# mahilab/mahi-mpc

Measured on AMD Instinct MI355X. Metric: MPC solves/sec (whole node), nx=4 N=30 batch, at 1/2/4/8 MI355X, higher is better.
Workload: dtype f64; 1 GPU; cfg#2: 2-link arm nx=4 nu=2, N=30, h=2 ms, cold-start SQP (exact or Gauss-Newton Hessian: config.hessian) to ||grad||<=1e-8, ||g||<=1e-10; batch_per_gpu=4096, global_batch=4096, horizon=30, kkt_solver=riccati (16 lanes per instance), hessian=exact (Lagrangian, IPOPT's default), init_states=reference cold start V = 0 (MMPC_INIT_ZERO: V not read)

## Files before the change

mahi-mpc_amd/csrc/mmpc.hip:

```cpp
#include <hip/hip_runtime.h>

#include <algorithm>
#include <atomic>
#include <cmath>
#include <cstdio>
#include <cstring>
#include <fstream>
#include <mutex>
#include <thread>
#include <sstream>
#include <string>
#include <type_traits>
#include <vector>

#include <dlfcn.h>
#include <rccl/rccl.h>

#include "../../include/mmpc.h"
#include "json_lite.h"
#include "adjoint_sweep.h"
#include "tangent_sweep.h"
#include "gain_sweep.h"
#include "group_launch.h"
#include "lane_launch.h"
// ... 591 lines not shown
        }
    }
    if (staged) {
        __syncthreads();
        const int64_t nb = B - b0 < I ? B - b0 : I;
        double* const dst = traj + b0 * N * 8;
        for (int t = threadIdx.x; t < nb * N * 8; t += kSynthThreads) dst[t] = so[t];
    }
}

inline unsigned grid1d(int64_t B, int threads) { return static_cast<unsigned>((B + threads - 1) / threads); }
inline unsigned synth_blocks(int64_t B, int N) {
    const int64_t I = N < kSynthThreads ? kSynthThreads / N : 1;
    return static_cast<unsigned>((B + I - 1) / I);
}

template <class F>
int with_model(int model_id, F&& f) {
#if MMPC_BUILTIN_MODELS
    if (model_id == MMPC_MODEL_TWO_LINK_ARM) return f(static_cast<TwoLinkArm*>(nullptr));
    if (model_id == MMPC_MODEL_EXO_ARM) return f(static_cast<ExoArm*>(nullptr));
#else
    if (model_id == MMPC_MODEL_USER) return f(static_cast<UserModel*>(nullptr));
#endif
    return fail(MMPC_ERR_UNSUPPORTED, "model not compiled into this library");
}
int model_nq(int model_id) {
    int nq = 0;
    with_model(model_id, [&](auto* m) {
        nq = std::remove_pointer_t<decltype(m)>::NQ;
        return MMPC_OK;
    });
    return nq;
}

mmpc_model_info with_horizon(const mmpc_model_info& mi, int N) {
    mmpc_model_info r = mi;
    r.num_shooting_nodes = N;
    r.num_v = mi.num_x * (N + 1) + mi.num_u * N;
    r.num_g = mi.num_x * N;
    return r;
}

int group_ws_doubles(const mmpc_model_info& mi, const KernelVariant& v) {
    return mmpc::group_ws_doubles(mi.num_x, mi.num_u, mi.num_shooting_nodes, v.ub, v.xb, false, v.mehr);
}
int lane_ws_doubles(const mmpc_model_info& mi, int nq, const KernelVariant& v) {
    return mmpc::lane_ws_doubles(mi.num_x, mi.num_u, nq, mi.num_shooting_nodes, v.xb);
}
size_t group_lds_instance_bytes(const mmpc_model_info& mi, int nq, const KernelVariant& v) {
    const int kc = mi.model_id == MMPC_MODEL_TWO_LINK_ARM ? mmpc::GroupLaneOps<TwoLinkArm>::doubles
                   : mi.model_id == MMPC_MODEL_EXO_ARM    ? mmpc::GroupLaneOps<ExoArm>::doubles
                                                          : 0;
    return static_cast<size_t>(mmpc::group_lds_doubles(mi.num_x, mi.num_u, nq, mi.num_shooting_nodes, v.ub,
                                                       mi.is_linear != 0, v.xb, kc)) * sizeof(double);
}
size_t group_lds_bytes(const mmpc_model_info& mi, int nq, const KernelVariant& v) {
    return group_lds_instance_bytes(mi, nq, v) * kGroupsPerWave;
}
constexpr size_t kMaxGroupLds = 160 * 1024;

size_t solver_workspace_bytes(const mmpc_model_info& mi, int nq, int64_t B) {
    const size_t lane = static_cast<size_t>(lane_ws_doubles(mi, nq, kVariantXb)) * 64u *
                        static_cast<size_t>((B + 63) / 64) * sizeof(double);
    const size_t group = static_cast<size_t>(std::max(group_ws_doubles(mi, kVariantUb),
                                                      group_ws_doubles(mi, kVariantXbMehrotra))) *
                         static_cast<size_t>(B) * sizeof(double);
    return (std::max(lane, group) + 255) / 256 * 256;
}

int resolve_kkt_solver_base(const mmpc_handle* h, int64_t B) {
    const mmpc_model_info& mi = h->info;
    if (h->opts.kkt_solver != MMPC_KKT_AUTO) return h->opts.kkt_solver;
    if (h->opts.factor_fp32) return MMPC_KKT_RICCATI;
    const int N = mi.num_shooting_nodes;
    const size_t glds = group_lds_bytes(mi, h->nq, h->x_bounded ? kVariantXb : kVariantUb);
    if (mi.model_id == MMPC_MODEL_USER) {
        if (glds <= kMaxGroupLds / 2 && B * static_cast<int64_t>(N) <= 1000000) return MMPC_KKT_RICCATI_GROUP;
        return MMPC_KKT_RICCATI;
    }
    if (mi.model_id == MMPC_MODEL_TWO_LINK_ARM) {
        if (N * TwoLinkArm::NU <= 64 && B <= 2560 && (h->opts.hessian == MMPC_HESSIAN_GAUSS_NEWTON || mi.is_linear))
            return MMPC_KKT_CONDENSED;
        if (glds <= kMaxGroupLds && B * static_cast<int64_t>(N) <= 1000000) return MMPC_KKT_RICCATI_GROUP;
        return MMPC_KKT_RICCATI;
    }
    if (glds <= kMaxGroupLds / 2 && B <= 4096) return MMPC_KKT_RICCATI_GROUP;
    return MMPC_KKT_RICCATI;
}
int resolve_kkt_solver(const mmpc_handle* h, int64_t B) {
    const int s = resolve_kkt_solver_base(h, B);
    if (h->x_bounded && h->opts.kkt_solver == MMPC_KKT_AUTO && s == MMPC_KKT_CONDENSED)
        return group_lds_bytes(h->info, h->nq, kVariantXb) <= kMaxGroupLds ? MMPC_KKT_RICCATI_GROUP : MMPC_KKT_RICCATI;
    return s;
}

template <class M>
constexpr bool exact_capable() {
    return HasHess<M>::value && (M::NX + M::NU < kGroupLanes);
}
template <class M, class = void>
struct ExactDefault {
    static constexpr bool value = true;
};
template <class M>
struct ExactDefault<M, std::enable_if_t<!M::kExactDefault || M::kExactDefault>> {
    static constexpr bool value = M::kExactDefault;
};
// ... 1826 lines not shown
```

mahi-mpc_amd/csrc/sqp_group.h:

```cpp
#undef MMPC_GROUP_PASS
#if defined(MMPC_GROUP_BODY_ONLY)
#define MMPC_GROUP_PASS 2
#elif !defined(MMPC_SQP_GROUP_H)
#define MMPC_SQP_GROUP_H
#define MMPC_GROUP_PASS 1
#else
#define MMPC_GROUP_PASS 0
#endif
#if MMPC_GROUP_PASS == 1
#include <type_traits>

#include "models.h"
#include "sqp_lane.h"
#include "sqp_wave.h"

namespace mmpc {

template <class Model>
__host__ __device__ constexpr bool w_struct_zero(int, int) { return false; }
template <>
__host__ __device__ constexpr bool w_struct_zero<TwoLinkArm>(int r, int j) { return (r == 0 && j >= 2) || (r >= 2 && (j == 0 || j >= 4)); }
template <class Model>
struct WPack {
    static constexpr int PK = 0, OVER = 0;
    __host__ __device__ static constexpr int col(int) { return 0; }
    __host__ __device__ static constexpr int idx(int, int) { return -1; }
};
template <>
struct WPack<TwoLinkArm> {
    static constexpr int PK = 10, OVER = 3;
    __host__ __device__ static constexpr int col(int i) { return i < 3 ? i : 2 * (i - 1); }
    __host__ __device__ static constexpr int idx(int r, int j) {
        if (w_struct_zero<TwoLinkArm>(r, j)) return -1;
        return col(r) + col(j);
    }
};
template <class Model>
__host__ __device__ constexpr bool wpack_valid() {
    using P = WPack<Model>;
    constexpr int NX = Model::NX, KZ = Model::NX + Model::NU;
    for (int r = 0; r < NX; ++r)
        for (int j = 0; j < KZ; ++j) {
            if (P::idx(r, j) < 0) continue;
            if (P::idx(r, j) >= P::PK || P::idx(r, j) != P::col(r) + P::col(j)) return false;
            for (int r2 = 0; r2 < NX; ++r2)
                for (int j2 = 0; j2 < KZ; ++j2)
                    if (P::idx(r2, j2) == P::idx(r, j) && !((r2 == r && j2 == j) || (r2 == j && j2 == r))) return false;
        }
    return P::OVER == P::col(NX - 1) + P::col(KZ - 1) - (P::PK - 1);
}
static_assert(wpack_valid<TwoLinkArm>(), "W record of the 2-link arm");
template <class Model>
__host__ __device__ constexpr int wpack_col_rep(int j) {
    for (int q = 0; q < j; ++q) {
        bool same = true;
        for (int r = 0; r < Model::NX; ++r) same = same && ((WPack<Model>::idx(r, q) < 0) == (WPack<Model>::idx(r, j) < 0));
        if (same) return q;
    }
    return j;
}
constexpr int kGroupLanes = 16;
constexpr int kGroupsPerWave = 4;

__host__ __device__ constexpr int group_const_doubles(int nx, int nu) {
    return nx + nu < kGroupLanes ? nx + (nx > nu ? nx : nu) : 0;
}
__host__ __device__ constexpr int group_lds_doubles(int nx, int nu, int nq, int N, bool bounded = true,
                                                   bool linear = true, bool xb = false, int kc = 0) {
    return N * (3 * nx + (nx - nq) * (nq + (nx - nq) + nu) + 2 * nu) + 3 * (N + 1) * nx + (bounded ? N * nu : 0) +
           (linear ? (nx - nq) * (nq + (nx - nq) + nu) + nx : 0) +
           (N * ((nx - nq) * nu + nx) >= 2 * (nx - nq) * (nx - nq) ? 0 : 2 * (nx - nq) * (nx - nq)) + kc;
}
template <class Model>
struct GroupLaneOps {
    static constexpr int doubles = 0;
};
template <>
struct GroupLaneOps<TwoLinkArm> {
    static constexpr int doubles = group_const_doubles(TwoLinkArm::NX, TwoLinkArm::NU);
};
__host__ __device__ constexpr int group_hess_doubles(int nx, int nu) { return nx * (nx + nu) + nu * nu; }
__host__ __device__ constexpr int group_ws_doubles(int nx, int nu, int N, bool bounded = true, bool xb = false,
                                                  bool w_onchip = false, bool mehr = false) {
    return N * nu * (nx + nu + 1) + (w_onchip ? 0 : N * group_hess_doubles(nx, nu)) +
           (bounded ? N * nu * (nx + 2 * nu + 1) : 0) + (xb ? 5 * N * (nx + nu) : 0) +
           (mehr ? 2 * N * (nx + nu) + N * ((2 + nu) * kGroupLanes + nu * (nu + 1) / 2 + nu) : 0);
}
static_assert(kGroupsPerWave * group_lds_doubles(4, 2, 2, 30, false, false, false, GroupLaneOps<TwoLinkArm>::doubles) * 8 <= 40960,
              "cfg#2 LDS budget");

struct GroupWork {
    double* ws;
};

template <int O>
__device__ __forceinline__ double row_ror(double v) {
    static_assert(O >= 1 && O < 16, "row rotation");
    return __builtin_amdgcn_update_dpp(v, v, 0x120 + O, 0xf, 0xf, true);
}
__device__ __forceinline__ double group_sum(double v) {
    v += row_ror<8>(v);
    v += row_ror<4>(v);
    v += row_ror<2>(v);
    v += row_ror<1>(v);
    return v;
}
__device__ __forceinline__ double group_min(double v) {
    v = fmin(v, row_ror<8>(v));
    v = fmin(v, row_ror<4>(v));
    v = fmin(v, row_ror<2>(v));
    v = fmin(v, row_ror<1>(v));
    return v;
}
__device__ __forceinline__ double group_max(double v) {
    v = fmax(v, row_ror<8>(v));
    v = fmax(v, row_ror<4>(v));
    v = fmax(v, row_ror<2>(v));
    v = fmax(v, row_ror<1>(v));
    return v;
}
__device__ __forceinline__ double group_bcast(double v, int base) { return __shfl(v, base); }
__device__ __forceinline__ int group_bcast_i(int v, int base) { return __shfl(v, base); }

template <int L>
__device__ __forceinline__ double row_bcast(double v) {
    static_assert(L >= 0 && L < 16, "row lane");
    return __builtin_amdgcn_update_dpp(v, v, 0x150 + L, 0xf, 0xf, true);
}
template <int B, int E, class F>
__device__ __forceinline__ void sfor(F&& f) {
    if constexpr (B < E) {
        f(std::integral_constant<int, B>{});
        sfor<B + 1, E>(static_cast<F&&>(f));
    }
}

template <class Model>
__device__ __forceinline__ void group_model(bool lin, const double* lFq, const double* lFqd, const double* lFu,
                                            const double* lxd, const double* lxs, const double* lus, const double* x,
                                            const double* u, double* xd, double* Fq, double* Fqd, double* Fu,
                                            bool jac) {
// ... 60 lines not shown
#pragma unroll
            for (int e = 0; e < W; ++e) {
#pragma unroll
                for (int i = 0; i < NQ; ++i) xd[e][i] = x[e][NQ + i];
#pragma unroll
                for (int i = 0; i < NA; ++i) xd[e][NQ + i] = xdw[NQ + i].v[e];
#pragma unroll
                for (int i = 0; i < NA * NQ; ++i) Fq[e][i] = fq[i].v[e];
#pragma unroll
                for (int i = 0; i < FD; ++i) Fqd[e][i] = fqd[i].v[e];
#pragma unroll
                for (int i = 0; i < FU; ++i) Fu[e][i] = fu[i].v[e];
            }
        } else {
            Model::eval(xw, uw, xdw);
#pragma unroll
            for (int e = 0; e < W; ++e)
#pragma unroll
                for (int i = 0; i < NX; ++i) xd[e][i] = xdw[i].v[e];
        }
    }
}

template <class Model, bool BOUNDED = false, bool XB = false, bool EXACT = false>
__global__ __launch_bounds__(64) void sqp_group_kernel(SolveParams p, GroupWork gw) {
    constexpr bool MEHR = false;
    constexpr bool IB = false;
#endif
#if MMPC_GROUP_PASS != 0
    static_assert(!(BOUNDED && XB), "the interior-point variant handles the control bounds itself");
    static_assert(!MEHR || XB, "the barrier rule belongs to the interior-point variant");
    constexpr int NX = Model::NX, NU = Model::NU, NQ = Model::NQ, NA = NX - NQ, NS = NX + NU, ND = NX + NU;
    constexpr int SQ = NA * NQ > 0 ? NA * NQ : 1;
    constexpr int FQ = NA * NQ, FD = NA * NA, FU = NA * NU;
    static_assert(NQ >= 0 && NA >= NQ, "x = [q; z] with qdot = z[0:NQ]");
    constexpr int G = kGroupLanes;
    extern __shared__ double shm[];
    const int gl = threadIdx.x & (G - 1);
    const int gi = threadIdx.x / G;
    [[maybe_unused]] const int lane0 = threadIdx.x;
    MMPC_PHASE_DECL
    const int gbase = gi * G;
    const int64_t slot = (int64_t)blockIdx.x * p.gpw + gi;
    const bool resume = p.tail_idx != nullptr;
    const bool valid = gi < p.gpw && slot < (resume ? (int64_t)min(*p.tail_count, p.tail_slots) : p.B);
    if (!valid) return;
    const int64_t inst = resume ? (int64_t)p.tail_idx[slot] : slot;
    const int64_t ii = inst;
    const int N = p.N;
    const int NV = NX * (N + 1) + NU * N;
    const double h = p.h;

    constexpr int KC = NX + NU < kGroupLanes ? GroupLaneOps<Model>::doubles : 0;
    double* const sX = shm + gi * group_lds_doubles(NX, NU, NQ, N, BOUNDED, p.is_linear != 0, XB, KC);
    double* const sU = sX + (N + 1) * NX;
    double* const sD = sU + N * NU;
    double* const sDX = sD + (N + 1) * NX;
    double* const sDU = sDX + (N + 1) * NX;
    double* const sF = sDU + N * NU;
    double* const sC = sF + N * NX;
    double* const sFq = sC + N * NX;
    double* const sFqd = sFq + N * FQ;
    double* const sFu = sFqd + N * FD;
    double* const sR = sFu + N * FU;
    double* const sHold = sR + N * NX;
    double* const sLin = sHold + (BOUNDED ? N * NU : 0);
    constexpr int NY = NX + NU;
    constexpr int PK = WPack<Model>::PK;
    constexpr bool WLDS = EXACT && !BOUNDED && !XB && IsControlAffine<Model>::value && PK >= NX && PK <= 2 * NX + NU;
    double* const wK = gw.ws + slot * (int64_t)group_ws_doubles(NX, NU, N, BOUNDED, XB, WLDS, MEHR);
    constexpr int KZ = NX + NU, HW = group_hess_doubles(NX, NU);
    double* const wH = wK + N * NU * (NS + 1);
    double* const sW = sD + NX;
    static_assert(!WLDS || WPack<Model>::OVER <= NX, "the over-read of the last W record stays inside sDU");
    if constexpr (WLDS) {
        if (gl < WPack<Model>::OVER) sW[N * PK + gl] = 0.0;
    }
    constexpr int NR = NS + NU + 1;
    double* const wRel = wH + N * HW;
    bool w_zeros_stored = false;
    double* const sZl = wRel;
    double* const sZu = sZl + N * NY;
    double* const sSg = sZu + N * NY;
    double* const sBb = sSg + N * NY;
    double* const sZg = sBb + N * NY;
    [[maybe_unused]] double* const sCl = sZg + N * NY;
    [[maybe_unused]] double* const sCu = sCl + N * NY;
    constexpr int VL = 2 + NU, VC = NU * (NU + 1) / 2, VS = VC + NU, VR = VL * G + VS;
    [[maybe_unused]] double* const sVr = sCu + N * NY;
    const double* const trg = p.traj + ii * (int64_t)N * NX;

    constexpr bool PAIR = HasWideEval<Model>::value && !BOUNDED && !XB;
    constexpr int WD = PAIR ? 2 : 1;
    constexpr int WA = WD, WJ = WD, WW = WD;
    const double* w = p.weights + ii * p.w_stride;
    double Q[NX], R[NU], Rm[NU], up[NU];
#pragma unroll
    for (int r = 0; r < NX; ++r) Q[r] = w[r];
#pragma unroll
    for (int c = 0; c < NU; ++c) {
        R[c] = w[NX + c];
        Rm[c] = w[NX + NU + c];
        up[c] = p.u_prev[ii * NU + c];
    }
    double lbv[NU], ubv[NU];
    load_bounds<NU, BOUNDED, IB>(p, inst, lbv, ubv);
    [[maybe_unused]] double px0[NX], pxv[WD][NX], puv[WD][NU], prv[WD][NX];
// ... 28 lines not shown
    if constexpr (PAIR) {
#pragma unroll
        for (int r = 0; r < NX; ++r) px0[r] = p.x0[ii * NX + r];
        pro_load(gl, pxv, puv, prv);
    }
    constexpr bool DIST = (NS < G);
    static_assert(!MEHR || DIST, "Mehrotra's rule: lane-distributed path");
    constexpr bool CAFF = IsControlAffine<Model>::value;
    static_assert(!EXACT || (DIST && HasHess<Model>::value), "exact Hessian: lane-distributed path, model eval_hess");
    const int r = gl;
    const bool lx = r < NX, lu = r >= NX && r < NS, la = r >= NQ && r < NX;
    const int rx = lx ? r : 0;
    const int ru = lu ? r - NX : 0;
    const int ta = la ? r - NQ : 0;
    const double Qr = lx ? w[rx] : 0.0;
    [[maybe_unused]] const double lqd = r < NQ ? 1.0 : 0.0, lad = la ? 1.0 : 0.0;
    const double lxf = lx ? 1.0 : 0.0;
    int wrow = 0;
#pragma unroll
    for (int r2 = 0; r2 < NX; ++r2)
        if (lx && r == r2) wrow = WPack<Model>::col(r2);
    double wm[KZ];
#pragma unroll
    for (int j = 0; j < KZ; ++j) {
        bool nz = false;
#pragma unroll
        for (int r2 = 0; r2 < NX; ++r2)
            if (lx && r == r2 && WPack<Model>::idx(r2, j) >= 0) nz = true;
        wm[j] = wpack_col_rep<Model>(j) < j ? wm[wpack_col_rep<Model>(j)] : (nz ? 1.0 : 0.0);
    }
    const int rq = r < NQ ? r : 0;
    const double Rr = lu ? w[NX + ru] : 0.0;
    double dgx[NS];
#pragma unroll
    for (int j = 0; j < NS; ++j) dgx[j] = (lx && j == r) ? 1.0 : 0.0;
    double lbr = -INFINITY, ubr = INFINITY;
#pragma unroll
    for (int c = 0; c < NU; ++c)
        if (lu && ru == c) {
            lbr = lbv[c];
            ubr = ubv[c];
        }
    double hq[NQ > 0 ? NQ : 1], hrow[NX], qoh[NX], rdg[NU];
#pragma unroll
    for (int z = 0; z < NQ; ++z) hq[z] = (r == NQ + z) ? h : 0.0;
#pragma unroll
    for (int j = 0; j < NX; ++j) {
        hrow[j] = (r < NQ && j == NQ + r) ? h : 0.0;
        qoh[j] = (j == r) ? Qr : 0.0;
    }
#pragma unroll
    for (int c = 0; c < NU; ++c) rdg[c] = (r == NX + c) ? R[c] : 0.0;
    constexpr bool LOPS = KC > 0;
    double* const sKc = sX + group_lds_doubles(NX, NU, NQ, N, BOUNDED, p.is_linear != 0, XB, KC) - KC;
    using LdsB = const __attribute__((address_space(3))) char*;
    using LdsD = const __attribute__((address_space(3))) double*;
    const LdsB shb = (LdsB)shm;
    auto lds = [](LdsB b) { return *(LdsD)b; };
    auto pin = [](LdsB& b) { asm volatile("" : "+v"(b)); };
    [[maybe_unused]] const LdsB iKc = shb + 8 * (int)(sKc - shm), iKz = iKc + 8 * NX;
    constexpr bool MIRROR = LOPS && NQ > 0 && NQ == NA && (NA - 1) * NA < KC;
    [[maybe_unused]] const double Qa = MIRROR ? w[rx] : Qr;
    [[maybe_unused]] const LdsB iAq =
        la ? shb + 8 * ((int)(sFq - shm) + ta * NQ) : ((r < NQ || MIRROR) ? iKc + 8 * ((NX - 1) - (NQ + rq)) : iKz);
    [[maybe_unused]] const int zAq = la ? 8 * FQ : 0, zAd = la ? 8 * FD : 0, zBr = la ? 8 * FU : 0;
    [[maybe_unused]] const LdsB iAd = la ? shb + 8 * ((int)(sFqd - shm) + ta * NA) : ((r < NQ || MIRROR) ? iAq + 8 * NQ : iKz);
    [[maybe_unused]] const LdsB iBr = la ? shb + 8 * ((int)(sFu - shm) + ta * NU) : iKz;
    constexpr bool ACOLP = LOPS && NQ == NA && (NA - 1) * NA < KC;
    static_assert(!MIRROR || ACOLP, "a mirrored lane reads row 0's column through the per-lane column address");
    [[maybe_unused]] const int zAc = (la || r < NQ) ? 8 * FD : 0;
    [[maybe_unused]] const LdsB iAc = la ? shb + 8 * ((int)(sFqd - shm) + ta) : (r < NQ ? shb + 8 * ((int)(sFq - shm) + rq) : iKc),
                                iAcN = iAc + (N - 1) * zAc;
    if constexpr (LOPS) {
        for (int i = gl; i < KC; i += G) sKc[i] = (i == NX - 1) ? h : 0.0;
    }
    if constexpr (PAIR) {
        const bool hold = p.init_hold != 0;
        for (int k0 = gl; k0 <= N; k0 += WD * G) {
            if (k0 != gl) pro_load(k0, pxv, puv, prv);
#pragma unroll
            for (int e = 0; e < WD; ++e) {
                const int k = pro_k(k0, e), ku = k < N ? k : N - 1;
#pragma unroll
                for (int r = 0; r < NX; ++r) sX[k * NX + r] = (k == 0 || hold) ? px0[r] : pxv[e][r];
#pragma unroll
                for (int c = 0; c < NU; ++c) sU[ku * NU + c] = puv[e][c];
#pragma unroll
                for (int r = 0; r < NX; ++r) sR[ku * NX + r] = prv[e][r];
            }
        }
    } else {
        const double* Vin = p.V + ii * (int64_t)NV;
        for (int k = gl; k <= N; k += G) {
#pragma unroll
            for (int r = 0; r < NX; ++r)
                sX[k * NX + r] = (k == 0 || p.init_hold) ? p.x0[ii * NX + r] : (p.init_zero ? 0.0 : Vin[k * ND + r]);
            if (k < N) {
#pragma unroll
                for (int c = 0; c < NU; ++c) {
                    const double v = p.init_zero ? 0.0 : Vin[k * ND + NX + c];
                    sU[k * NU + c] = BOUNDED ? proj(v, lbv[c], ubv[c]) : v;
                }
#pragma unroll
                for (int r = 0; r < NX; ++r) sR[k * NX + r] = trg[k * NX + r];
            }
        }
    }
// ... 709 lines not shown
                for (int c = 0; c < NU; ++c) {
                    double g = 0.0;
#pragma unroll
                    for (int s2 = 0; s2 < NA; ++s2) g = fma(sFu[k * FU + s2 * NU + c], sD[(k + 1) * NX + NQ + s2], g);
                    const double uk = sU[k * NU + c], um = k == 0 ? up[c] : sU[(k - 1) * NU + c];
                    g = fma(R[c], uk - um, fma(Rm[c], uk, g));
                    if (k < N - 1) g -= R[c] * (sU[(k + 1) * NU + c] - uk);
                    if constexpr (XB) g += sZg[k * NY + NX + c];
                    if constexpr (!BOUNDED) {
                        gmax = fmax(gmax, fabs(2.0 * g));
                    } else {
                        gmax = fmax(gmax, fabs(uk - proj(uk - 2.0 * g, lbv[c], ubv[c])));
                        sHold[k * NU + c] = (uk <= lbv[c] + beps && g > 0.0)   ? lbv[c]
                                            : (uk >= ubv[c] - beps && g < 0.0) ? ubv[c]
                                                                                : NAN;
                    }
                    nonfinite |= !isfinite(g);
                }
            }
        };
        auto backward_dist = [&](bool useW) {
            if constexpr (BOUNDED) {
                __builtin_amdgcn_fence(__ATOMIC_RELEASE, "workgroup");
                __builtin_amdgcn_fence(__ATOMIC_ACQUIRE, "workgroup");
            }
            double Prow[NS], pvr;
            [[maybe_unused]] LdsB jcol = iAcN;
            const double lxm = lx ? 1.0 : 0.0;
            struct Wb {
                double r[KZ], u[NU * NU];
            };
            Wb w0;
            auto load_w = [&](int k, Wb& b) {
#pragma unroll
                for (int j = 0; j < KZ; ++j)
                    b.r[j] = WLDS ? sW[k * PK + wrow + WPack<Model>::col(j)] : wH[k * HW + rx * KZ + j];
                if constexpr (!CAFF) {
#pragma unroll
                    for (int j = 0; j < NU * NU; ++j) b.u[j] = wH[k * HW + NX * KZ + j];
                }
            };
            if (EXACT && useW) {
                load_w(N - 1, w0);
            }
#pragma unroll
            for (int j = 0; j < NS; ++j) Prow[j] = j < NX ? qoh[j] : 0.0;
            pvr = Qr * (lx ? sX[N * NX + rx] - tr[(N - 1) * NX + rx] : 0.0);
            if constexpr (XB) {
                const double sgN = sSg[(N - 1) * NY + rx], bbN = sBb[(N - 1) * NY + rx];
#pragma unroll
                for (int j = 0; j < NX; ++j) Prow[j] = fma(dgx[j], sgN, Prow[j]);
                pvr = fma(lxm, bbN, pvr);
            }
            auto stage = [&](int k, auto last_c, Wb& wb) {
                constexpr bool LAST = decltype(last_c)::value;
#if defined(MMPC_PHASE_TIMING) && defined(MMPC_PHASE_STAGES)
                if (gl == 0 && blockIdx.x < kPhaseWavePhases && k < 32)
                    g_mmpc_phase_cycles[kPhaseStageLog + 128 * blockIdx.x + 32 * gi + k] = __builtin_amdgcn_s_memtime();
#endif
                double hFq[SQ], hFqd[FD], hFu[FU], cc[NX], u[NU], um[NU], acol[NA];
#pragma unroll
                for (int i = 0; i < FQ; ++i) hFq[i] = sFq[k * FQ + i];
#pragma unroll
                for (int i = 0; i < FD; ++i) hFqd[i] = sFqd[k * FD + i];
#pragma unroll
                for (int i = 0; i < FU; ++i) hFu[i] = sFu[k * FU + i];
#pragma unroll
                for (int q = 0; q < NX; ++q) cc[q] = sC[k * NX + q];
#pragma unroll
                for (int c = 0; c < NU; ++c) {
                    u[c] = sU[k * NU + c];
                    um[c] = LAST ? up[c] : sU[(k - 1) * NU + c];
                }
                load_acol(k, jcol, acol);
                double xsgu[XB ? NU : 1], xbbu[XB ? NU : 1], xsgx = 0.0, xbbx = 0.0;
                if constexpr (XB) {
#pragma unroll
                    for (int a = 0; a < NU; ++a) {
                        xsgu[a] = sSg[k * NY + NX + a];
                        xbbu[a] = sBb[k * NY + NX + a];
                    }
                    if constexpr (!LAST) {
                        xsgx = sSg[(k - 1) * NY + rx];
                        xbbx = sBb[(k - 1) * NY + rx];
                    }
                }
                double exr = 0.0, duu = 0.0;
                if constexpr (!LAST) {
                    const double xk = sX[k * NX + rx], trm = tr[(k - 1) * NX + rx];
                    exr = xk - trm;
                    duu = sU[k * NU + ru] - sU[(k - 1) * NU + ru];
                }
                double wr[KZ], wu[NU * NU];
                if constexpr (EXACT) {
#pragma unroll
                    for (int j = 0; j < KZ; ++j) wr[j] = useW ? wb.r[j] : 0.0;
#pragma unroll
                    for (int j = 0; j < NU * NU; ++j) wu[j] = (useW && !CAFF) ? wb.u[j] : 0.0;
                    if (!LAST && useW) load_w(k - 1, wb);
                }
                double T[NU], mv = pvr;
#pragma unroll
                for (int b = 0; b < NU; ++b) {
                    double t = Prow[NX + b];
#pragma unroll
                    for (int s2 = 0; s2 < NA; ++s2) t = fma(Prow[NQ + s2], hFu[s2 * NU + b], t);
                    T[b] = t;
                }
#pragma unroll
                for (int q = 0; q < NX; ++q) mv = fma(Prow[q], cc[q], mv);
                double Tb[NS][NU], mvb[NS];
                sfor<0, NS>([&](auto I) {
#pragma unroll
                    for (int b = 0; b < NU; ++b) Tb[I][b] = row_bcast<I>(T[b]);
                    mvb[I] = row_bcast<I>(mv);
                });
                double Hww[NU][NU], hw[NU];
#pragma unroll
                for (int a = 0; a < NU; ++a) {
#pragma unroll
                    for (int b = a; b < NU; ++b) {
                        double t = Tb[NX + a][b];
#pragma unroll
                        for (int s2 = 0; s2 < NA; ++s2) t = fma(hFu[s2 * NU + a], Tb[NQ + s2][b], t);
                        if (a == b) t += R[a] + Rm[a];
                        if constexpr (EXACT && !CAFF) t += wu[a * NU + b];
                        if constexpr (XB) {
// ... 142 lines not shown
                    double Ld[NU][NU], il[NU];
#pragma unroll
                    for (int a = 0; a < NU; ++a) {
                        double sd = Hww[a][a];
#pragma unroll
                        for (int q = 0; q < a; ++q) sd = fma(-Ld[a][q], Ld[a][q], sd);
                        fact_ok &= (sd > 0.0) && isfinite(sd);
                        const double sp = fmax(sd, 1e-300);
                        double rr = __builtin_amdgcn_rsq(sp);
                        rr = rr * fma(-0.5 * sp * rr, rr, 1.5);
                        rr = rr * fma(-0.5 * sp * rr, rr, 1.5);
                        Ld[a][a] = sp * rr;
                        il[a] = rr;
#pragma unroll
                        for (int b = a + 1; b < NU; ++b) {
                            double t = Hww[a][b];
#pragma unroll
                            for (int q = 0; q < a; ++q) t = fma(-Ld[b][q], Ld[a][q], t);
                            Ld[b][a] = t * il[a];
                        }
                    }
                    auto chol_solve = [&](const double* rhs, double* out) {
                        double y[NU];
#pragma unroll
                        for (int a = 0; a < NU; ++a) {
                            double t = rhs[a];
#pragma unroll
                            for (int q = 0; q < a; ++q) t = fma(-Ld[a][q], y[q], t);
                            y[a] = t * il[a];
                        }
#pragma unroll
                        for (int a = NU - 1; a >= 0; --a) {
                            double t = y[a];
#pragma unroll
                            for (int q = a + 1; q < NU; ++q) t = fma(-Ld[q][a], out[q], t);
                            out[a] = t * il[a];
                        }
                    };
                    chol_solve(Ycol, Kcol);
                    chol_solve(hw, kff);
#pragma unroll
                    for (int c = 0; c < NU; ++c) {
                        double e[NU], o[NU];
#pragma unroll
                        for (int a = 0; a < NU; ++a) e[a] = (a == c) ? -Rk[c] : 0.0;
                        chol_solve(e, o);
#pragma unroll
                        for (int a = 0; a < NU; ++a) Ku[a][c] = o[a];
                    }
                }
                {
                    const int col = r < NS ? r : NS;
#pragma unroll
                    for (int a = 0; a < NU; ++a) wK[(k * NU + a) * (NS + 1) + col] = -(r < NS ? Kcol[a] : kff[a]);
                }
                if constexpr (LAST) return;
                double Pb[NX][NX];
                sfor<0, NX>([&](auto I) {
#pragma unroll
                    for (int j = I; j < NX; ++j) {
                        Pb[I][j] = row_bcast<I>(Prow[j]);
                        Pb[j][I] = Pb[I][j];
                    }
                });
                double Ur[NX], Pn[NX];
#pragma unroll
                for (int j = 0; j < NX; ++j) {
                    double pc[NX];
#pragma unroll
                    for (int q = 0; q < NX; ++q) pc[q] = Pb[q][j];
                    Ur[j] = colA(Prow[j], acol, pc);
                }
                at_mul<NQ, NA, double>(h, hFq, hFqd, Ur, Pn);
                double pn = fma(-Rr, duu, lxm * fma(Qr, exr, colA(mv, acol, mvb)));
                double sgk = 0.0;
                if constexpr (XB) {
                    sgk = xsgx;
                    pn = fma(lxm, xbbx, pn);
                }
                if constexpr (XB) {
                    double Yb[NU][NS];
                    sfor<0, NS>([&](auto I) {
#pragma unroll
                        for (int a = 0; a < NU; ++a) Yb[a][I] = row_bcast<I>(Ytil[a]);
                    });
#pragma unroll
                    for (int j = 0; j < NS; ++j) {
                        double v = j < NX ? fma(dgx[j], sgk, Pn[j] + qoh[j]) : rdg[j - NX];
                        if constexpr (EXACT) {
                            if (j < NX) v = fma(lxm, wr[j], v);
                        }
#pragma unroll
                        for (int a = 0; a < NU; ++a) v = fma(-Ytil[a], Yb[a][j], v);
                        Prow[j] = v;
                    }
                    double pv2 = pn;
#pragma unroll
                    for (int a = 0; a < NU; ++a) pv2 = fma(-Ytil[a], htil[a], pv2);
                    pvr = pv2;
                    return;
                }
                double Kb[NU][NX];
                sfor<0, NX>([&](auto I) {
#pragma unroll
                    for (int a = 0; a < NU; ++a) Kb[a][I] = row_bcast<I>(Kcol[a]);
                });
#pragma unroll
                for (int j = 0; j < NS; ++j) {
                    double v = j < NX ? Pn[j] + qoh[j] : rdg[j - NX];
                    if constexpr (EXACT) {
                        if (j < NX) v = fma(WLDS ? wm[j] : lxm, wr[j], v);
                    }
#pragma unroll
                    for (int a = 0; a < NU; ++a) v = fma(-Ycol[a], j < NX ? Kb[a][j] : Ku[a][j - NX], v);
                    Prow[j] = v;
                }
                double pv2 = pn;
#pragma unroll
                for (int a = 0; a < NU; ++a) pv2 = fma(-Ycol[a], kff[a], pv2);
                if constexpr (BOUNDED) pv2 += pexr;
                pvr = pv2;
            };
            using F_ = std::false_type;
            if constexpr (BOUNDED || (XB && EXACT)) {
                for (int k = N - 1; k >= 1; --k) stage(k, F_{}, w0);
                stage(0, std::true_type{}, w0);
            } else if ((N - 1) & 1) {
                stage(N - 1, F_{}, w0);
                for (int k = N - 2; k >= 2; k -= 2) {
                    stage(k, F_{}, w0);
                    stage(k - 1, F_{}, w0);
                }
                stage(0, std::true_type{}, w0);
            } else {
                for (int k = N - 1; k >= 2; k -= 2) {
                    stage(k, F_{}, w0);
                    stage(k - 1, F_{}, w0);
                }
                stage(0, std::true_type{}, w0);
            }
        };
        [[maybe_unused]] auto backward_vec = [&]() {
            if constexpr (MEHR) {
                const double lxm = lx ? 1.0 : 0.0;
                [[maybe_unused]] LdsB jcol = iAcN;
                double pvr = Qr * (lx ? sX[N * NX + rx] - tr[(N - 1) * NX + rx] : 0.0);
                pvr = fma(lxm, sBb[(N - 1) * NY + rx], pvr);
                struct Rec {
                    double pc, pn0, yt[NU], sh[VS], bbu[NU], bbx;
                };
                auto fetch = [&](int k, Rec& o) {
                    const double* const rec = sVr + k * VR;
                    o.pc = rec[r];
                    o.pn0 = rec[G + r];
#pragma unroll
                    for (int a = 0; a < NU; ++a) {
                        o.yt[a] = rec[(2 + a) * G + r];
                        o.bbu[a] = sBb[k * NY + NX + a];
                    }
#pragma unroll
                    for (int i = 0; i < VS; ++i) o.sh[i] = rec[VL * G + i];
                    o.bbx = sBb[(k > 0 ? k - 1 : 0) * NY + rx];
                };
                auto stage = [&](int k, const Rec& o) {
                    double hFu[FU], acol[NA];
#pragma unroll
                    for (int i = 0; i < FU; ++i) hFu[i] = sFu[k * FU + i];
                    load_acol(k, jcol, acol);
                    const double mv = pvr + o.pc;
                    double mvb[NS];
                    sfor<0, NS>([&](auto I) { mvb[I] = row_bcast<I>(mv); });
                    double htil[NU], kff[NU];
#pragma unroll
                    for (int a = 0; a < NU; ++a) {
                        double t = o.sh[VC + a] + mvb[NX + a];
#pragma unroll
                        for (int s2 = 0; s2 < NA; ++s2) t = fma(hFu[s2 * NU + a], mvb[NQ + s2], t);
                        t += o.bbu[a];
#pragma unroll
                        for (int q = 0; q < a; ++q) t = fma(-o.sh[a * (a + 1) / 2 + q], htil[q], t);
                        htil[a] = t * o.sh[a * (a + 1) / 2 + a];
                    }
#pragma unroll
                    for (int a = NU - 1; a >= 0; --a) {
                        double t = htil[a];
#pragma unroll
                        for (int q = a + 1; q < NU; ++q) t = fma(-o.sh[q * (q + 1) / 2 + a], kff[q], t);
                        kff[a] = t * o.sh[a * (a + 1) / 2 + a];
                    }
#pragma unroll
                    for (int a = 0; a < NU; ++a) wK[(k * NU + a) * (NS + 1) + NS] = -kff[a];
                    if (k == 0) return;
// ... 146 lines not shown
                        if constexpr (!CAFF) {
#pragma unroll
                            for (int a = 0; a < NU; ++a)
#pragma unroll
                                for (int b = 0; b < NU; ++b) dst[NX * KZ + a * NU + b] = W[e][(NX + a) * KZ + NX + b];
                        }
                    }
                }
            };
            auto w_pair = [&](int k0) {
                int kk[WW];
#pragma unroll
                for (int e = 0; e < WW; ++e) kk[e] = (e == 0 || k0 + e * G < N) ? k0 + e * G : k0;
                w_stages(kk);
            };
            if constexpr (WLDS) {
                for (int k0 = ((N - 1) / (WW * G)) * (WW * G); k0 >= 0; k0 -= WW * G)
                    if (k0 + gl < N) w_pair(k0 + gl);
                MMPC_PHASE(9);
                __builtin_amdgcn_wave_barrier();
            } else {
                for (int k = gl; k < N; k += WW * G) w_pair(k);
                w_zeros_stored = true;
                MMPC_PHASE(9);
                __builtin_amdgcn_fence(__ATOMIC_RELEASE, "workgroup");
                __builtin_amdgcn_fence(__ATOMIC_ACQUIRE, "workgroup");
            }
        }
        bool use_w = EXACT;
        if constexpr (DIST) {
            backward_dist(use_w);
            if (EXACT && !fact_ok) {
                fact_ok = 1;
                use_w = false;
                backward_dist(false);
            }
        }
        if (!fact_ok) {
            status = ST_FACT_FAILED;
            break;
        }
        if (BOUNDED) pg_prev = gmax;
        const double mub_next = (XB && fmax(fmax(0.5 * gmax, cmax), cmplmu) <= kIpKappaEps * mub)
                                    ? fmax(kIpTolCompl / 20.0, fmin(kIpKappaMu * mub, pow(mub, kIpThetaMu)))
                                    : mub;

        MMPC_PHASE(3);
        if constexpr (DIST) {
            auto step_dist = [&](bool check) {
                __builtin_amdgcn_fence(__ATOMIC_RELEASE, "workgroup");
                __builtin_amdgcn_fence(__ATOMIC_ACQUIRE, "workgroup");
                constexpr bool RUN = MIRROR;
                double sr = 0.0;
                if (RUN || lx) sDX[rx] = 0.0;
                constexpr int NK = NS + 1;
                const double* const Kp = wK + ru * NK;
                struct Ops {
                    double K[NK], a[NX], b[NU], c, Rw[BOUNDED ? NR : 1];
                };
                const double* const Rp = wRel + ru * NR;
                using LdsW = __attribute__((address_space(3))) double*;
                [[maybe_unused]] LdsB ja = iAq, jd = iAd, jb = iBr, jcs = shb + 8 * ((int)(sC - shm) + rx);
                [[maybe_unused]] LdsB js = shb + 8 * (lu ? (int)(sDU - shm) + ru : (int)(sDX - shm) + NX + rx);
                [[maybe_unused]] LdsB jt = shb + 8 * (lu ? (int)(sD - shm) + ru : (int)(sD - shm) + NX + rx);
                [[maybe_unused]] const int zs = lu ? 8 * NU : 8 * NX, zt = lu ? 0 : 8 * NX;
                using GlbD = const __attribute__((address_space(1))) double*;
                [[maybe_unused]] GlbD jK = (GlbD)Kp;
                [[maybe_unused]] GlbD jR = (GlbD)Rp;
                [[maybe_unused]] auto refill = [&](Ops& o) {
#pragma unroll
                    for (int j = 0; j < NK; ++j) o.K[j] = jK[j];
#pragma unroll
                    for (int s2 = 0; s2 < NQ; ++s2) o.a[s2] = lds(ja + 8 * s2);
#pragma unroll
                    for (int s2 = 0; s2 < NA; ++s2) o.a[NQ + s2] = lds(jd + 8 * s2);
#pragma unroll
                    for (int c = 0; c < NU; ++c) o.b[c] = lds(jb + 8 * c);
                    o.c = lds(jcs);
                    if constexpr (BOUNDED) {
#pragma unroll
                        for (int j = 0; j < NR; ++j) o.Rw[j] = jR[j];
                    }
                };
                [[maybe_unused]] auto advance = [&]() {
                    ja += zAq;
                    jd += zAd;
                    jb += zBr;
                    jcs += 8 * NX;
                    jK += NU * NK;
                    pin(ja);
                    pin(jd);
                    pin(jb);
                    pin(jcs);
                    asm volatile("" : "+v"(jK));
                    if constexpr (BOUNDED) {
                        jR += NU * NR;
                        asm volatile("" : "+v"(jR));
                    }
                };
                auto fetch = [&](int k, Ops& o) {
#pragma unroll
                    for (int j = 0; j < NK; ++j) o.K[j] = Kp[k * NU * NK + j];
                    load_arow(k, o.a, o.b);
                    o.c = sC[k * NX + rx];
                    if constexpr (BOUNDED) {
#pragma unroll
                        for (int j = 0; j < NR; ++j) o.Rw[j] = Rp[k * NU * NR + j];
                    }
                };
                auto stage = [&](int k, Ops& o, [[maybe_unused]] bool more = true) {
                    double sb[NS];
                    sfor<0, NS>([&](auto I) { sb[I] = row_bcast<I>(sr); });
                    double du0 = o.K[NS], du1 = 0.0;
#pragma unroll
                    for (int j = 0; j < NS; ++j) {
                        if (j & 1) du1 = fma(o.K[j], sb[j], du1);
                        else du0 = fma(o.K[j], sb[j], du0);
                    }
                    const double du = du0 + du1;
                    double ad = sr;
#pragma unroll
                    for (int j = 0; j < NX; ++j) ad = fma(o.a[j], sb[j], ad);
                    double dub[NU];
                    sfor<0, NU>([&](auto I) { dub[I] = row_bcast<NX + I>(du); });
#pragma unroll
                    for (int c = 0; c < NU; ++c) ad = fma(o.b[c], dub[c], ad);
                    const double dxn = ad + o.c;
                    if constexpr (RUN) {
                        sr = lu ? du : dxn;
                        *(LdsW)js = sr;
                        *(LdsW)jt = ad;
                        js += zs;
                        jt += zt;
                        pin(js);
                        pin(jt);
                    } else {
                        if (lx) {
                            sDX[(k + 1) * NX + rx] = dxn;
                            sD[(k + 1) * NX + rx] = ad;
                        }
                        if (lu) sDU[k * NU + ru] = du;
                    }
                    if constexpr (BOUNDED) {
                        if (check && lu) {
                            const double hv = sHold[k * NU + ru], t = sU[k * NU + ru] + du;
                            if (hv != hv) {
                                if (t < lbr || t > ubr) {
                                    sHold[k * NU + ru] = t < lbr ? lbr : ubr;
                                    resolve = true;
                                }
                            } else if (!p.no_release) {
                                double m = o.Rw[NR - 1];
#pragma unroll
                                for (int j = 0; j < NS; ++j) m = fma(o.Rw[j], sb[j], m);
#pragma unroll
                                for (int b = 0; b < NU; ++b) m = fma(o.Rw[NS + b], dub[b], m);
                                if ((hv == lbr && m < 0.0) || (hv == ubr && m > 0.0)) {
                                    sHold[k * NU + ru] = NAN;
                                    resolve = true;
                                }
                            }
                        }
                    }
                    if constexpr (RUN) {
                        if (more) {
                            refill(o);
                            advance();
                        }
                    } else {
                        sr = lx ? dxn : (lu ? du : 0.0);
                        fetch(k + 3 < N ? k + 3 : N - 1, o);
                    }
                };
                Ops o0, o1, o2;
                if constexpr (RUN) {
                    refill(o0);
                    if (N > 1) advance();
                    refill(o1);
                    if (N > 2) advance();
                    refill(o2);
                    advance();
                    int k = 0;
                    for (; k + 5 < N; k += 3) {
                        stage(k, o0, true);
                        stage(k + 1, o1, true);
                        stage(k + 2, o2, true);
                    }
                    const int left = N - 3 - k;
                    if (left == 1) {
                        stage(k, o0, true);
                        stage(k + 1, o1, false);
                        stage(k + 2, o2, false);
                        stage(k + 3, o0, false);
                    } else if (left == 2) {
                        stage(k, o0, true);
                        stage(k + 1, o1, true);
                        stage(k + 2, o2, false);
                        stage(k + 3, o0, false);
                        stage(k + 4, o1, false);
                    } else {
                        stage(k, o0, false);
                        if (N >= 2) stage(k + 1, o1, false);
                        if (N >= 3) stage(k + 2, o2, false);
                    }
                    return;
                }
                fetch(0, o0);
                fetch(N > 1 ? 1 : 0, o1);
                fetch(N > 2 ? 2 : 0, o2);
                if (N % 3 == 1) {
                    stage(0, o0);
                    for (int k = 1; k < N; k += 3) {
                        stage(k, o1);
                        stage(k + 1, o2);
                        stage(k + 2, o0);
                    }
                } else if (N % 3 == 2) {
                    stage(0, o0);
                    stage(1, o1);
                    for (int k = 2; k < N; k += 3) {
                        stage(k, o2);
                        stage(k + 1, o0);
                        stage(k + 2, o1);
                    }
                } else {
                    for (int k = 0; k < N; k += 3) {
                        stage(k, o0);
                        stage(k + 1, o1);
                        stage(k + 2, o2);
                    }
                }
            };
            if constexpr (MEHR) {
                step_dist(false);
// ... 376 lines not shown
```

mahi-mpc_amd/csrc/sqp_wave.h:

```cpp
#pragma once
#include <hip/hip_runtime.h>
#include <stdint.h>

#include "models.h"

#ifndef MMPC_WAVES_PER_SIMD
#define MMPC_WAVES_PER_SIMD 2
#endif

namespace mmpc {

struct SolveParams {
    int64_t B;
    int N;
    int max_iter;
    double h;
    double tol_grad;
    double tol_defect;
    int is_linear;
    const double* x0;
    const double* u_prev;
    const double* traj;
    const double* weights;
    int64_t w_stride;
// ... 266 lines not shown
    return lg;
}

#define MMPC_PIN(x) asm volatile("" : "+v"(x))
__device__ __forceinline__ double readlane_d(double v, int l) {
    const int lo = __builtin_amdgcn_readlane(__double2loint(v), l);
    const int hi = __builtin_amdgcn_readlane(__double2hiint(v), l);
    return __hiloint2double(hi, lo);
}

template <int CTRL>
__device__ __forceinline__ double dpp_d(double v) {
    const int lo = __builtin_amdgcn_mov_dpp(__double2loint(v), CTRL, 0xF, 0xF, false);
    const int hi = __builtin_amdgcn_mov_dpp(__double2hiint(v), CTRL, 0xF, 0xF, false);
    return __hiloint2double(hi, lo);
}
template <int Q>
__device__ __forceinline__ double quad_bcast(double v) {
    return dpp_d<Q | (Q << 2) | (Q << 4) | (Q << 6)>(v);
}
template <int S>
__device__ __forceinline__ double row_rot4(double v) {
    return dpp_d<0x120 + 4 * S>(v);
}
template <int S>
__device__ __forceinline__ int row_rot4_src(int lane) {
    return __builtin_amdgcn_mov_dpp(lane, 0x120 + 4 * S, 0xF, 0xF, false);
}

__device__ __forceinline__ double wave_sum(double v) {
#pragma unroll
    for (int o = 32; o >= 1; o >>= 1) v += __shfl_xor(v, o);
    return v;
}
__device__ __forceinline__ double wave_max(double v) {
#pragma unroll
    for (int o = 32; o >= 1; o >>= 1) v = fmax(v, __shfl_xor(v, o));
    return v;
}

__device__ __forceinline__ double rcp_nr(double a) {
    double r = __builtin_amdgcn_rcp(a);
    double e = fma(-a, r, 1.0);
    r = fma(r, e, r);
    e = fma(-a, r, 1.0);
    return fma(r, e, r);
}

constexpr int kPhaseWaveLog = 4096;
constexpr int kPhaseWavePhases = 1024;
constexpr int kPhaseStageLog = 16 + 2 * kPhaseWaveLog + 40 * kPhaseWavePhases;
constexpr int kPhaseSpread = 64;
constexpr int kPhaseSpreadBase = kPhaseStageLog + 128 * kPhaseWavePhases;
constexpr int kPhaseSlots = kPhaseSpreadBase + 32 * kPhaseSpread;
#ifdef MMPC_PHASE_TIMING
constexpr int kPhaseTableSlots = kPhaseSlots;
#else
constexpr int kPhaseTableSlots = 16;
#endif
__device__ unsigned long long g_mmpc_phase_cycles[kPhaseTableSlots];
static inline hipError_t phase_table_read(unsigned long long* out, int n, bool reset) {
    static unsigned long long full[kPhaseTableSlots];
    hipError_t e = hipMemcpyFromSymbol(full, HIP_SYMBOL(g_mmpc_phase_cycles), sizeof(full));
    if (e != hipSuccess) return e;
#ifdef MMPC_PHASE_TIMING
    for (int c = 0; c < kPhaseSpread; ++c)
        for (int q = 0; q < 16; ++q) {
            const unsigned long long v = full[kPhaseSpreadBase + 32 * c + q];
            full[q] = (q >= 10 && q <= 12) ? (v > full[q] ? v : full[q]) : full[q] + v;
        }
#endif
    for (int i = 0; i < n; ++i) out[i] = full[i];
    if (reset) {
        static const unsigned long long z[kPhaseTableSlots] = {0};
        e = hipMemcpyToSymbol(HIP_SYMBOL(g_mmpc_phase_cycles), z, sizeof(z));
    }
    return e;
}
#ifdef MMPC_PHASE_TIMING
#define MMPC_PHASE_DECL                                                                            \
    unsigned long long ph_acc[10] = {0}, ph_t = __builtin_amdgcn_s_memtime(), ph_m0 = ph_t,        \
                       ph_r0 = __builtin_amdgcn_s_memrealtime();
#define MMPC_PHASE(i)                                        \
    do {                                                     \
        __builtin_amdgcn_sched_barrier(0);                   \
        const unsigned long long t_ = __builtin_amdgcn_s_memtime(); \
        ph_acc[i] += t_ - ph_t;                              \
        ph_t = t_;                                           \
        __builtin_amdgcn_sched_barrier(0);                   \
    } while (0)
#define MMPC_PHASE_FLUSH                                                                   \
    if (lane0 == 0) {                                                                      \
        const unsigned long long r1_ = __builtin_amdgcn_s_memrealtime(),                   \
                                 m1_ = __builtin_amdgcn_s_memtime();                       \
        unsigned long long* const pc_ = g_mmpc_phase_cycles + kPhaseSpreadBase + 32 * (blockIdx.x % kPhaseSpread); \
        for (int q_ = 0; q_ < 10; ++q_) atomicAdd(&pc_[q_], ph_acc[q_]);                   \
        atomicMax(&pc_[10], r1_);                                                          \
        atomicMax(&pc_[11], ~ph_r0);                                                       \
        atomicMax(&pc_[12], r1_ - ph_r0);                                                  \
        atomicAdd(&pc_[13], r1_ - ph_r0);                                                  \
        atomicAdd(&pc_[14], m1_ - ph_m0);                                                  \
        atomicAdd(&pc_[15], 1ull);                                                         \
        if (blockIdx.x < kPhaseWaveLog) {                                                  \
            g_mmpc_phase_cycles[16 + blockIdx.x] = r1_ - ph_r0;                            \
            g_mmpc_phase_cycles[16 + kPhaseWaveLog + blockIdx.x] = m1_ - ph_m0;            \
        }                                                                                  \
    }                                                                                      \
// ... 641 lines not shown
```

Baseline: 31.88 million solves/s.

## Prefetch next-stage head operands in Riccati backward sweep and keep first gains in LDS

In the group Riccati backward sweep, the Fu and C operands for stage k-1 are now loaded into registers during stage k, so the load overlaps compute instead of stalling at the start of each stage. The Fq and Fqd loads move after the acol load. The gains for the last three stages (k=0..2) are written to a new LDS region instead of global workspace, and the forward rollout reads its first refills from there, which avoids a global round trip at the backward-to-forward handoff. This costs extra LDS per group (checked by the static_assert), more register pressure, and phase-timing instrumentation that is compiled only under debug defines.

```diff
diff --git a/mahi-mpc_amd/csrc/mmpc.hip b/mahi-mpc_amd/csrc/mmpc.hip
--- a/mahi-mpc_amd/csrc/mmpc.hip
+++ b/mahi-mpc_amd/csrc/mmpc.hip
@@ -667,8 +667,9 @@
     const int kc = mi.model_id == MMPC_MODEL_TWO_LINK_ARM ? mmpc::GroupLaneOps<TwoLinkArm>::doubles
                    : mi.model_id == MMPC_MODEL_EXO_ARM    ? mmpc::GroupLaneOps<ExoArm>::doubles
                                                           : 0;
+    const int kh = kc > 0 && !v.ub && !v.xb ? mmpc::group_head_doubles(mi.num_x, mi.num_u) : 0;
     return static_cast<size_t>(mmpc::group_lds_doubles(mi.num_x, mi.num_u, nq, mi.num_shooting_nodes, v.ub,
-                                                       mi.is_linear != 0, v.xb, kc)) * sizeof(double);
+                                                       mi.is_linear != 0, v.xb, kc, kh)) * sizeof(double);
 }
 size_t group_lds_bytes(const mmpc_model_info& mi, int nq, const KernelVariant& v) {
     return group_lds_instance_bytes(mi, nq, v) * kGroupsPerWave;
diff --git a/mahi-mpc_amd/csrc/sqp_group.h b/mahi-mpc_amd/csrc/sqp_group.h
--- a/mahi-mpc_amd/csrc/sqp_group.h
+++ b/mahi-mpc_amd/csrc/sqp_group.h
@@ -65,11 +65,12 @@
 __host__ __device__ constexpr int group_const_doubles(int nx, int nu) {
     return nx + nu < kGroupLanes ? nx + (nx > nu ? nx : nu) : 0;
 }
+__host__ __device__ constexpr int group_head_doubles(int nx, int nu) { return 3 * nu * (nx + nu + 1); }
 __host__ __device__ constexpr int group_lds_doubles(int nx, int nu, int nq, int N, bool bounded = true,
-                                                   bool linear = true, bool xb = false, int kc = 0) {
+                                                   bool linear = true, bool xb = false, int kc = 0, int kh = 0) {
     return N * (3 * nx + (nx - nq) * (nq + (nx - nq) + nu) + 2 * nu) + 3 * (N + 1) * nx + (bounded ? N * nu : 0) +
            (linear ? (nx - nq) * (nq + (nx - nq) + nu) + nx : 0) +
-           (N * ((nx - nq) * nu + nx) >= 2 * (nx - nq) * (nx - nq) ? 0 : 2 * (nx - nq) * (nx - nq)) + kc;
+           (N * ((nx - nq) * nu + nx) >= 2 * (nx - nq) * (nx - nq) ? 0 : 2 * (nx - nq) * (nx - nq)) + kh + kc;
 }
 template <class Model>
 struct GroupLaneOps {
@@ -86,7 +87,8 @@
            (bounded ? N * nu * (nx + 2 * nu + 1) : 0) + (xb ? 5 * N * (nx + nu) : 0) +
            (mehr ? 2 * N * (nx + nu) + N * ((2 + nu) * kGroupLanes + nu * (nu + 1) / 2 + nu) : 0);
 }
-static_assert(kGroupsPerWave * group_lds_doubles(4, 2, 2, 30, false, false, false, GroupLaneOps<TwoLinkArm>::doubles) * 8 <= 40960,
+static_assert(kGroupsPerWave * group_lds_doubles(4, 2, 2, 30, false, false, false, GroupLaneOps<TwoLinkArm>::doubles,
+                                                 group_head_doubles(4, 2)) * 8 <= 40960,
               "cfg#2 LDS budget");
 
 struct GroupWork {
@@ -253,7 +255,8 @@
     const double h = p.h;
 
     constexpr int KC = NX + NU < kGroupLanes ? GroupLaneOps<Model>::doubles : 0;
-    double* const sX = shm + gi * group_lds_doubles(NX, NU, NQ, N, BOUNDED, p.is_linear != 0, XB, KC);
+    constexpr int KH = (KC > 0 && !BOUNDED && !XB) ? group_head_doubles(NX, NU) : 0;
+    double* const sX = shm + gi * group_lds_doubles(NX, NU, NQ, N, BOUNDED, p.is_linear != 0, XB, KC, KH);
     double* const sU = sX + (N + 1) * NX;
     double* const sD = sU + N * NU;
     double* const sDX = sD + (N + 1) * NX;
@@ -388,7 +391,8 @@
 #pragma unroll
     for (int c = 0; c < NU; ++c) rdg[c] = (r == NX + c) ? R[c] : 0.0;
     constexpr bool LOPS = KC > 0;
-    double* const sKc = sX + group_lds_doubles(NX, NU, NQ, N, BOUNDED, p.is_linear != 0, XB, KC) - KC;
+    double* const sKc = sX + group_lds_doubles(NX, NU, NQ, N, BOUNDED, p.is_linear != 0, XB, KC, KH) - KC;
+    [[maybe_unused]] double* const sKh = sKc - KH;
     using LdsB = const __attribute__((address_space(3))) char*;
     using LdsD = const __attribute__((address_space(3))) double*;
     const LdsB shb = (LdsB)shm;
@@ -1204,27 +1208,59 @@
                 for (int j = 0; j < NX; ++j) Prow[j] = fma(dgx[j], sgN, Prow[j]);
                 pvr = fma(lxm, bbN, pvr);
             }
-            auto stage = [&](int k, auto last_c, Wb& wb) {
-                constexpr bool LAST = decltype(last_c)::value;
+            struct Hb {
+                double fu[FU], c[NX];
+            };
+            Hb h0;
+            auto load_head = [&](int k, Hb& b) {
+#pragma unroll
+                for (int i = 0; i < FU; ++i) b.fu[i] = sFu[k * FU + i];
+#pragma unroll
+                for (int q = 0; q < NX; ++q) b.c[q] = sC[k * NX + q];
+            };
+            if constexpr (LOPS) load_head(N - 1, h0);
+            auto stage = [&](int k, auto last_c, auto head_c, Wb& wb, Hb& hb) {
+                constexpr bool LAST = decltype(last_c)::value, HEADK = decltype(head_c)::value;
 #if defined(MMPC_PHASE_TIMING) && defined(MMPC_PHASE_STAGES)
-                if (gl == 0 && blockIdx.x < kPhaseWavePhases && k < 32)
-                    g_mmpc_phase_cycles[kPhaseStageLog + 128 * blockIdx.x + 32 * gi + k] = __builtin_amdgcn_s_memtime();
+                const unsigned long long st_top = __builtin_amdgcn_s_memtime();
+                __builtin_amdgcn_sched_barrier(0);
 #endif
                 double hFq[SQ], hFqd[FD], hFu[FU], cc[NX], u[NU], um[NU], acol[NA];
-#pragma unroll
-                for (int i = 0; i < FQ; ++i) hFq[i] = sFq[k * FQ + i];
-#pragma unroll
-                for (int i = 0; i < FD; ++i) hFqd[i] = sFqd[k * FD + i];
-#pragma unroll
-                for (int i = 0; i < FU; ++i) hFu[i] = sFu[k * FU + i];
-#pragma unroll
-                for (int q = 0; q < NX; ++q) cc[q] = sC[k * NX + q];
+                if constexpr (!LOPS) {
+#pragma unroll
+                    for (int i = 0; i < FQ; ++i) hFq[i] = sFq[k * FQ + i];
+#pragma unroll
+                    for (int i = 0; i < FD; ++i) hFqd[i] = sFqd[k * FD + i];
+                    load_head(k, hb);
+                }
+#pragma unroll
+                for (int i = 0; i < FU; ++i) hFu[i] = hb.fu[i];
+#pragma unroll
+                for (int q = 0; q < NX; ++q) cc[q] = hb.c[q];
+#if defined(MMPC_PHASE_TIMING) && defined(MMPC_PHASE_STAGES)
+#pragma unroll
+                for (int i = 0; i < FU; ++i) asm volatile("" ::"v"(hFu[i]));
+#pragma unroll
+                for (int q = 0; q < NX; ++q) asm volatile("" ::"v"(cc[q]));
+                __builtin_amdgcn_sched_barrier(0);
+                if (gl == 0 && blockIdx.x < kPhaseWavePhases && k < 32) {
+                    g_mmpc_phase_cycles[kPhaseStageLog + 128 * blockIdx.x + 32 * gi + k] = st_top;
+                    g_mmpc_phase_cycles[kPhaseWaitLog + 128 * blockIdx.x + 32 * gi + k] = __builtin_amdgcn_s_memtime();
+                }
+                __builtin_amdgcn_sched_barrier(0);
+#endif
 #pragma unroll
                 for (int c = 0; c < NU; ++c) {
                     u[c] = sU[k * NU + c];
                     um[c] = LAST ? up[c] : sU[(k - 1) * NU + c];
                 }
                 load_acol(k, jcol, acol);
+                if constexpr (LOPS) {
+#pragma unroll
+                    for (int i = 0; i < FQ; ++i) hFq[i] = sFq[k * FQ + i];
+#pragma unroll
+                    for (int i = 0; i < FD; ++i) hFqd[i] = sFqd[k * FD + i];
+                }
                 double xsgu[XB ? NU : 1], xbbu[XB ? NU : 1], xsgx = 0.0, xbbx = 0.0;
                 if constexpr (XB) {
 #pragma unroll
@@ -1473,7 +1509,8 @@
                 {
                     const int col = r < NS ? r : NS;
 #pragma unroll
-                    for (int a = 0; a < NU; ++a) wK[(k * NU + a) * (NS + 1) + col] = -(r < NS ? Kcol[a] : kff[a]);
+                    for (int a = 0; a < NU; ++a)
+                        (HEADK ? sKh : wK)[(k * NU + a) * (NS + 1) + col] = -(r < NS ? Kcol[a] : kff[a]);
                 }
                 if constexpr (LAST) return;
                 double Pb[NX][NX];
@@ -1493,6 +1530,10 @@
                     Ur[j] = colA(Prow[j], acol, pc);
                 }
                 at_mul<NQ, NA, double>(h, hFq, hFqd, Ur, Pn);
+                if constexpr (LOPS) {
+                    load_head(k - 1, hb);
+                    __builtin_amdgcn_sched_barrier(0);
+                }
                 double pn = fma(-Rr, duu, lxm * fma(Qr, exr, colA(mv, acol, mvb)));
                 double sgk = 0.0;
                 if constexpr (XB) {
@@ -1543,22 +1584,37 @@
                 pvr = pv2;
             };
             using F_ = std::false_type;
+            using T_ = std::true_type;
             if constexpr (BOUNDED || (XB && EXACT)) {
-                for (int k = N - 1; k >= 1; --k) stage(k, F_{}, w0);
-                stage(0, std::true_type{}, w0);
+                for (int k = N - 1; k >= 1; --k) stage(k, F_{}, F_{}, w0, h0);
+                stage(0, T_{}, F_{}, w0, h0);
+            } else if constexpr (KH > 0) {
+                int k = N - 1;
+                if (N >= 4 && ((N - 3) & 1)) stage(k--, F_{}, F_{}, w0, h0);
+                for (; k >= 4; k -= 2) {
+                    stage(k, F_{}, F_{}, w0, h0);
+                    stage(k - 1, F_{}, F_{}, w0, h0);
+                }
+                if (N >= 3) {
+                    stage(2, F_{}, T_{}, w0, h0);
+                    stage(1, F_{}, T_{}, w0, h0);
+                } else if (N == 2) {
+                    stage(1, F_{}, T_{}, w0, h0);
+                }
+                stage(0, T_{}, T_{}, w0, h0);
             } else if ((N - 1) & 1) {
-                stage(N - 1, F_{}, w0);
+                stage(N - 1, F_{}, F_{}, w0, h0);
                 for (int k = N - 2; k >= 2; k -= 2) {
-                    stage(k, F_{}, w0);
-                    stage(k - 1, F_{}, w0);
-                }
-                stage(0, std::true_type{}, w0);
+                    stage(k, F_{}, F_{}, w0, h0);
+                    stage(k - 1, F_{}, F_{}, w0, h0);
+                }
+                stage(0, T_{}, F_{}, w0, h0);
             } else {
                 for (int k = N - 1; k >= 2; k -= 2) {
-                    stage(k, F_{}, w0);
-                    stage(k - 1, F_{}, w0);
-                }
-                stage(0, std::true_type{}, w0);
+                    stage(k, F_{}, F_{}, w0, h0);
+                    stage(k - 1, F_{}, F_{}, w0, h0);
+                }
+                stage(0, T_{}, F_{}, w0, h0);
             }
         };
         [[maybe_unused]] auto backward_vec = [&]() {
@@ -1811,6 +1867,10 @@
                 __builtin_amdgcn_fence(__ATOMIC_ACQUIRE, "workgroup");
                 constexpr bool RUN = MIRROR;
                 double sr = 0.0;
+#if defined(MMPC_PHASE_TIMING) && defined(MMPC_PHASE_STAGES)
+                if (gl == 0 && blockIdx.x < kPhaseWavePhases)
+                    g_mmpc_phase_cycles[kPhaseStepLog + 8 * blockIdx.x + 2 * gi] = __builtin_amdgcn_s_memtime();
+#endif
                 if (RUN || lx) sDX[rx] = 0.0;
                 constexpr int NK = NS + 1;
                 const double* const Kp = wK + ru * NK;
@@ -1826,9 +1886,9 @@
                 using GlbD = const __attribute__((address_space(1))) double*;
                 [[maybe_unused]] GlbD jK = (GlbD)Kp;
                 [[maybe_unused]] GlbD jR = (GlbD)Rp;
-                [[maybe_unused]] auto refill = [&](Ops& o) {
-#pragma unroll
-                    for (int j = 0; j < NK; ++j) o.K[j] = jK[j];
+                [[maybe_unused]] auto refill = [&](Ops& o, int hs = -1) {
+#pragma unroll
+                    for (int j = 0; j < NK; ++j) o.K[j] = (KH > 0 && hs >= 0) ? sKh[(hs * NU + ru) * NK + j] : jK[j];
 #pragma unroll
                     for (int s2 = 0; s2 < NQ; ++s2) o.a[s2] = lds(ja + 8 * s2);
 #pragma unroll
@@ -1921,6 +1981,11 @@
                             }
                         }
                     }
+#if defined(MMPC_PHASE_TIMING) && defined(MMPC_PHASE_STAGES)
+                    asm volatile("" ::"v"(sr), "v"(ad));
+                    if (k == 0 && gl == 0 && blockIdx.x < kPhaseWavePhases)
+                        g_mmpc_phase_cycles[kPhaseStepLog + 8 * blockIdx.x + 2 * gi + 1] = __builtin_amdgcn_s_memtime();
+#endif
                     if constexpr (RUN) {
                         if (more) {
                             refill(o);
@@ -1933,12 +1998,21 @@
                 };
                 Ops o0, o1, o2;
                 if constexpr (RUN) {
-                    refill(o0);
-                    if (N > 1) advance();
-                    refill(o1);
-                    if (N > 2) advance();
-                    refill(o2);
-                    advance();
+                    if (KH == 0 || N < 3) {
+                        refill(o0, 0);
+                        if (N > 1) advance();
+                        refill(o1, N > 1 ? 1 : 0);
+                        if (N > 2) advance();
+                        refill(o2, N > 2 ? 2 : N - 1);
+                        advance();
+                    } else {
+                        refill(o0, 0);
+                        advance();
+                        refill(o1, 1);
+                        advance();
+                        refill(o2, 2);
+                        advance();
+                    }
                     int k = 0;
                     for (; k + 5 < N; k += 3) {
                         stage(k, o0, true);
diff --git a/mahi-mpc_amd/csrc/sqp_wave.h b/mahi-mpc_amd/csrc/sqp_wave.h
--- a/mahi-mpc_amd/csrc/sqp_wave.h
+++ b/mahi-mpc_amd/csrc/sqp_wave.h
@@ -342,7 +342,9 @@
 constexpr int kPhaseStageLog = 16 + 2 * kPhaseWaveLog + 40 * kPhaseWavePhases;
 constexpr int kPhaseSpread = 64;
 constexpr int kPhaseSpreadBase = kPhaseStageLog + 128 * kPhaseWavePhases;
-constexpr int kPhaseSlots = kPhaseSpreadBase + 32 * kPhaseSpread;
+constexpr int kPhaseWaitLog = kPhaseSpreadBase + 32 * kPhaseSpread;
+constexpr int kPhaseStepLog = kPhaseWaitLog + 128 * kPhaseWavePhases;
+constexpr int kPhaseSlots = kPhaseStepLog + 8 * kPhaseWavePhases;
 #ifdef MMPC_PHASE_TIMING
 constexpr int kPhaseTableSlots = kPhaseSlots;
 #else
```

Measured after the change: 33.01 million solves/s (median of 6 runs). +3.5%, better.
